# lppllppl920/EndoscopyDepthEstimation-Pytorch

Measured on AMD Instinct MI355X. Metric: train frame-pairs/sec at 256x320 bs=8, higher is better.
Workload: dtype f32

## Files before the change

endoscopydepthestimation-pytorch_amd/csrc/conv_dma_kernels.h:

```cpp
#pragma once

#include "conv_kernels.h"

namespace endo {

static __device__ __attribute__((aligned(16))) float g_pad_consts[8] = {__builtin_nanf(""), __builtin_nanf(""), __builtin_nanf(""), __builtin_nanf(""),
                                                                  0.0f, 0.0f, 0.0f, 0.0f};

typedef const __attribute__((address_space(1))) void* gptr_t;
typedef __attribute__((address_space(3))) void* lptr_t;

template <int KS, int KC, int Q, int WX, int R, int NBUF, int VEC, int IN = IN_PLAIN>
struct ConvDmaSmem {
    using G = ConvGeom<KS, KC, WX, R, VEC>;
    static constexpr int kW = KS * KS * KC * 16 * Q;
    static constexpr int kUG = (G::kTileX / 2) * (G::kTileY / 2);
    static constexpr int kUI = kUG / 4;
    static constexpr int kUStride = ((kUG + kUI - 8 + 31) / 32) * 32 + 8;
    static constexpr int kChan = (IN == IN_UNPOOL) ? kUStride : G::kCS;
    static constexpr int kBuf = KC * kChan + kW;
    static constexpr int kTail = 4 * 16 * Q + 8 * 16 * Q;
    static size_t bytes(int bn_cap) { return sizeof(float) * (NBUF * kBuf + 3 * bn_cap + kTail); }
};

// ... 613 lines not shown
    return launch_dyn(conv_dma_kernel<KS, KC, Q, IN, EPI, WX, R, NBUF, MINW, VEC, XF, EXP, PH, BF>, grid, kConvThreads, S::bytes(p.bn_cap), stream, p);
}

template <int KS, int KC, int Q, int IN, int EPI, int WX, int R, int NBUF, int MINW = 1, int BF = 0>
inline int launch_conv_dma(const ConvParams& p, hipStream_t stream) {
    if constexpr (IN != IN_UPSAMPLE && IN != IN_UNPOOL) {
        const bool aligned = (p.w % 4 == 0) && (p.in_w % 4 == 0) && (p.in_cs % 4 == 0) && (p.in_ns % 4 == 0) &&
                             (reinterpret_cast<uintptr_t>(p.in) % 16 == 0);
        if (aligned) return launch_conv_dma_vec<KS, KC, Q, IN, EPI, WX, R, NBUF, MINW, 4, 0, 0, -1, BF>(p, stream);
    }
    return launch_conv_dma_vec<KS, KC, Q, IN, EPI, WX, R, NBUF, MINW, 1, 0, 0, -1, BF>(p, stream);
}

template <int KS, int KC, int Q, int IN, int EPI, int BIG_R = 8, int NBUF = 2, int BIG_MINW = 1, int BF = 0>
inline int launch_conv_dma_auto(const ConvParams& p, hipStream_t stream) {
    const long tiles_big = static_cast<long>((p.w + 31) / 32) * ((p.h + 15) / 16) * p.n;
    if (tiles_big >= 512) return launch_conv_dma<KS, KC, Q, IN, EPI, 2, BIG_R, NBUF, BIG_MINW, BF>(p, stream);
    const long tiles_mid = static_cast<long>((p.w + 15) / 16) * ((p.h + 15) / 16) * p.n;
    if (tiles_mid >= 384) return launch_conv_dma<KS, KC, Q, IN, EPI, 1, 4, NBUF, 1, BF>(p, stream);
    constexpr int KCS = (NBUF == 2 && KS == 3 && KC <= 8) ? 16 : KC;
    return launch_conv_dma<KS, KCS, Q, IN, EPI, 1, 2, NBUF, 1, BF>(p, stream);
}

}
```

endoscopydepthestimation-pytorch_amd/csrc/conv_kernels.h:

```cpp
#pragma once

#include "common.h"

namespace endo {

enum InMode { IN_PLAIN = 0, IN_BNRELU = 1, IN_UPSAMPLE = 2, IN_UNPOOL = 3, IN_SUBPIX = 4 };
enum Epilogue { EPI_FWD = 0, EPI_FWD_POOL = 1, EPI_DGRAD_BN = 2, EPI_DGRAD_SUMPOOL = 3 };

constexpr int kConvThreads = 256;
constexpr int kMaxBnChannels = 384;

struct ConvParams {
    int n, h, w;
    int tiles_x;
    const float* in;
    int64_t in_ns;
    int in_cs;
    int in_w;
    const uint8_t* in_idx;
    int64_t idx_ns;
    int cin;
    const double* in_sums;
    const float* gamma;
    const float* beta;
// ... 18 lines not shown
    int x_cs;
    const float* bn_saved;
    const float* bn_gamma;
    const float* bn_beta;
    double* bn_scratch;
    int64_t bn_slot_stride;
    int acc_from;
    int bn_cap;
    int ksplit;
    int64_t split_stride;
    int group_n;
    int64_t gs, in_gs, out_gs;
    int sub_c;
    const float* fin_w;
    float* fin_out;
};

__device__ __forceinline__ void group_of(const ConvParams& p, int z, int& grp, int& n) {
    grp = p.group_n > 0 ? z / p.group_n : 0;
    n = z - grp * p.group_n;
}

__device__ __forceinline__ ConvParams group_view(const ConvParams& p, int grp) {
    ConvParams q = p;
    const int64_t o = grp * p.gs;
    q.in += grp * p.in_gs;
    q.out += grp * p.out_gs;
    if (q.x) q.x += o;
    if (q.in_idx) q.in_idx += 4 * o;
    if (q.out_idx) q.out_idx += 4 * o;
    if (q.in_sums) q.in_sums += o / 2;
    if (q.out_sums) q.out_sums += o / 2;
    if (q.bn_scratch) q.bn_scratch += o / 2;
    if (q.saved) q.saved += o;
    if (q.bn_saved) q.bn_saved += o;
    return q;
}

__device__ __forceinline__ void bn_input_constants(const ConvParams& p, const ConvParams& p0, int grp, int groups, bool first_of_group,
                                                   int c, float& scale, float& mean_f, float& beta) {
    double mean, var;
    if (p.training) {
        mean = p.in_sums[2 * c] / p.count;
        var = p.in_sums[2 * c + 1] / p.count - mean * mean;
        if (var < 0.0) var = 0.0;
    } else {
        mean = p.running_mean[c];
        var = p.running_var[c];
    }
    const double rstd = 1.0 / sqrt(var + static_cast<double>(p.eps));
    scale = p.gamma[c] * static_cast<float>(rstd);
    mean_f = static_cast<float>(mean);
    beta = p.beta[c];
    if (first_of_group) {
        if (p.saved) {
            p.saved[2 * c] = static_cast<float>(mean);
            p.saved[2 * c + 1] = static_cast<float>(rstd);
        }
        if (p.training && grp == 0) {
            float rm = p.running_mean[c], rv = p.running_var[c];
            for (int g = 0; g < groups; ++g) {
                const double* sums = p0.in_sums + g * (p0.gs / 2);
                const double m = sums[2 * c] / p.count;
                double v = sums[2 * c + 1] / p.count - m * m;
                if (v < 0.0) v = 0.0;
                const double unbiased = p.count > 1.0 ? v * p.count / (p.count - 1.0) : v;
                rm = (1.0f - p.momentum) * rm + p.momentum * static_cast<float>(m);
                rv = (1.0f - p.momentum) * rv + p.momentum * static_cast<float>(unbiased);
            }
            p.running_mean[c] = rm;
            p.running_var[c] = rv;
        }
    }
}

typedef float f32x4 __attribute__((ext_vector_type(4)));

template <int KS, int KC, int WX, int R, int VEC = 1>
struct ConvGeom {
    static constexpr int kTileX = 16 * WX;
    static constexpr int kTileY = R * (4 / WX);
    static constexpr int kHalo = KS / 2;
    static constexpr int kRows = kTileY + 2 * kHalo;
    static constexpr int kLeft = (VEC == 4 && KS == 3) ? 4 : kHalo;
    static constexpr int kCols = kTileX + 2 * kLeft;
    static constexpr int kColOff = kLeft - kHalo;
    static constexpr int kPlane = kRows * kCols;
// ... 421 lines not shown
```

endoscopydepthestimation-pytorch_amd/csrc/net.hip:

```cpp
#include <new>
#include <vector>

#include "dgrad_kernels.h"
#include "dgrad_block_kernels.h"
#include "dgrad_newmap_kernels.h"
#include "td_dgrad_kernels.h"
#include "td_fwd_kernels.h"
#include "wgrad_taps_kernels.h"
#include "wgrad1x1_kernels.h"
#include "wgrad_nsplit_kernels.h"
#include "wgrad_x3_kernels.h"
#include "wgrad_f34_kernels.h"
#include "wgrad_subpix_kernels.h"
#include "wino_fwd_kernels.h"
#include "wino4_fwd_kernels.h"
#include "dgrad_wino_kernels.h"
#include "dgrad_wino3_kernels.h"


namespace endo {

int run_dgrad_wino3_nl4(const DgradBlockParams& p, const float* const* u, hipStream_t stream);
bool dgrad_wino3p_applies(const DgradBlockParams& p);
int run_dgrad_wino3p_nl4(const DgradBlockParams& p, const float* const* u, int blocks, double* fw_parts, int* blocks_used, hipStream_t stream);

constexpr int kGrowth = 12;
constexpr int kLayers = 4;
constexpr int kFirst = 48;
constexpr int kLevels = 5;
constexpr int kNew = kGrowth * kLayers;
constexpr float kBnEps = 1.0e-5f;
constexpr float kBnMomentum = 0.1f;
constexpr int kSideStreamFromLevel = 0;

struct ConvP { int64_t w, b; int cout, cin, ks; int64_t u; int64_t ud; };
struct BnP { int64_t g, b; int c; int64_t run; int64_t saved; };

struct Table {
    ConvP first, final_;
    ConvP down_conv[kLevels][kLayers], td_conv[kLevels], bott_conv[kLayers], tu_conv[kLevels], up_conv[kLevels][kLayers];
    BnP down_bn[kLevels][kLayers], td_bn[kLevels], bott_bn[kLayers], up_bn[kLevels][kLayers];
    std::vector<int64_t> param_offsets;
    std::vector<BnP*> bn_order;
    int64_t param_floats = 0, bn_floats = 0, bn_width_total = 0;
    WinoWeightTable wino;
    WinoWeightTable wino4;
    int64_t wino4_floats = 0;
// ... 84 lines not shown

struct endo_net {
    int n, h, w;
    int groups;
    int64_t gs;
    struct Level { int h, w, t; int64_t plane; int64_t act, grad; int64_t sums; int64_t pq; } lv[kLevels + 1];
    int64_t pre_off;
    int64_t saved_off;
    int64_t idx_off[kLevels];
    int64_t sums_off;
    int64_t sums_bytes;
    int64_t tape_floats;
    int64_t partial_off;
    int64_t wino_off;
    int64_t wino4_off;
    int64_t pq_off;
    int64_t pq_floats;
    int64_t scratch_off;
    int64_t scratch_bytes;
    int64_t slot_stride;
    int64_t wg_scratch_off;
    int64_t tuw_scratch_off;
    int64_t wd_off;
    int64_t gplane_off;
    int64_t bias_parts_off;
    int64_t fw_parts_off;
    int64_t bias_parts_floats;
    int64_t gradws_floats;
    hipStream_t wstream;
    hipEvent_t ev_fork, ev_join;
// ... 160 lines not shown
            if (training) {
                const double mean = a.saved[j][go + 2 * c], rstd = a.saved[j][go + 2 * c + 1];
                const double scale = a.gamma[j][c] * rstd;
                const double k = scale * rstd * s2 / count;
                dp += static_cast<double>(static_cast<float>(-k));
                dq += static_cast<double>(static_cast<float>(-scale * s1 / count + k * mean));
            }
        }
        if (training) {
            pq_p[c] += static_cast<float>(dp);
            pq_q[c] += static_cast<float>(dq);
        }
    }
}

__global__ void tu_phase_weights_kernel(const float* __restrict__ w, int cout, int cin, float* __restrict__ out) {
    constexpr int kPhW = 2 * 12 * 16 + 16;
    const int total = 2 * cin * 2 * 12 * 16;
    for (int i = blockIdx.x * blockDim.x + threadIdx.x; i < total; i += gridDim.x * blockDim.x) {
        const int lane16 = i & 15;
        const int slot = (i >> 4) % 12;
        const int t = (i / (16 * 12)) & 1;
        const int ci = (i / (16 * 12 * 2)) % cin;
        const int a = i / (16 * 12 * 2 * cin);
        int ctap, tile;
        if (slot < 3) { ctap = 0; tile = slot; } else if (slot < 9) { ctap = 1; tile = slot - 3; } else { ctap = 2; tile = slot - 9 + 3; }
        const int b = tile / 3, co = (tile % 3) * 16 + lane16;
        float v = 0.f;
        if (co < cout) {
            const float* src = w + (static_cast<int64_t>(co) * cin + ci) * 9;
            const int ky0 = a == 0 ? (t == 0 ? 0 : 1) : (t == 0 ? 0 : 2), ky1 = a == 0 ? (t == 0 ? 0 : 2) : (t == 0 ? 1 : 2);
            int kx0, kx1;
// ... 11 lines not shown
    const int total = 4 * cout * 4 * cin;
    for (int i = blockIdx.x * blockDim.x + threadIdx.x; i < total; i += gridDim.x * blockDim.x) {
        const int ci = i % cin;
        const int tap = (i / cin) & 3;
        const int co = (i / (4 * cin)) % cout;
        const int ph = i / (4 * cin * cout);
        const int alpha = ph >> 1, beta = ph & 1, tyi = tap >> 1, txi = tap & 1;
        const int ky0 = alpha == 0 ? (tyi == 0 ? 1 : 0) : (tyi == 0 ? 2 : 0), ky1 = alpha == 0 ? (tyi == 0 ? 2 : 0) : (tyi == 0 ? 2 : 1);
        const int kx0 = beta == 0 ? (txi == 0 ? 1 : 0) : (txi == 0 ? 2 : 0), kx1 = beta == 0 ? (txi == 0 ? 2 : 0) : (txi == 0 ? 2 : 1);
        const float* src = w + (static_cast<int64_t>(co) * cin + ci) * 9;
        float v = 0.f;
        for (int ky = ky0; ky <= ky1; ++ky)
            for (int kx = kx0; kx <= kx1; ++kx) v += src[ky * 3 + kx];
        out[static_cast<int64_t>(ph * cout + co) * pitch + tap * cin + ci] = v;
    }
}

__global__ void __launch_bounds__(256) finalize_partial_kernel(const float* __restrict__ partial, int64_t split_stride, int ksplit,
                                                               int64_t pns, int plane, const float* __restrict__ bias,
                                                               float* __restrict__ out, int64_t out_ns, double* out_sums,
                                                               int group_n, int64_t gs) {
    __shared__ double scratch[2 * 4];
    const int c = blockIdx.y;
    const int grp = blockIdx.z / group_n, n = blockIdx.z - grp * group_n;
    partial += grp * gs; out += grp * gs;
    if (out_sums) out_sums += grp * (gs / 2);
    const float b = bias[c];
    float part[2] = {0.f, 0.f};
    for (int i = blockIdx.x * blockDim.x + threadIdx.x; i < plane; i += gridDim.x * blockDim.x) {
        float v = b;
// ... 112 lines not shown
constexpr int kBlocks = 2 * kLevels + 1, kDense = kBlocks * kLayers;

enum class DenseFwd { Wino4, Wino2_32x16, Wino2_32x8, SplitK, Direct32x8, Direct16x8, DirectAuto };
struct FwdPlan {
    struct Dense {
        DenseFwd form;
        int stages;
        int ksplit;
        bool chunk_weights;
    } dense[kDense];
    bool bf16;
    bool wino4_weights;
    bool fuse_final;
    bool td_persistent[kLevels];
    bool tu_subpix[kLevels];
};

enum class NewMap { Bf16, Persistent, Vec16, Dword };
enum class BasePass { Block8, Block8Bf16, Wino3, Wino3Persistent, Wino8 };
enum class DenseWgrad { F34, X3, NSplit, Taps, Direct };
enum class TdDgrad { Persistent, Runs128, Dma, Staged };
enum class TuWgrad { Subpix, Taps, Direct };
enum class TuDgrad { Subpix32x8, Subpix16x8, Subpix16x4, Plain };
enum class FirstWgrad { F34Prep, F34, Taps, Direct };
struct BwdPlan {
    struct Block {
        bool fused;
        NewMap newmap[kLayers];
        BasePass base;
        bool wino3_layout;
// ... 16 lines not shown
};

struct Ctx {
    const endo_net* net;
    const float* params;
    float* bn_running;
    float* tape;
    float* grads;
    float* gradws;
    int training;
    hipStream_t stream;
    BiasParts* bias_parts = nullptr;
    const float* x = nullptr;
    const FwdPlan* fwd = nullptr;
    const BwdPlan* bwd = nullptr;

    int nt() const { return net->n * net->groups; }
    int fork_wgrad(Ctx& side, int level) const {
        side = *this;
        if (!net->wstream || !bwd->overlap || level < kSideStreamFromLevel) return 0;
        ENDO_CHECK(hipEventRecord(net->ev_fork, stream));
        ENDO_CHECK(hipStreamWaitEvent(net->wstream, net->ev_fork, 0));
        side.stream = net->wstream;
        return 0;
    }
    float* act(int level) const { return tape + net->lv[level].act; }
    float* gbuf(int level) const { return gradws + net->lv[level].grad; }
    double* sums(int level) const { return reinterpret_cast<double*>(reinterpret_cast<char*>(tape) + net->sums_off) + net->lv[level].sums; }
    double* out_sums(int level, int channel) const { return training ? sums(level) + 2 * channel : nullptr; }
    float* saved(const BnP& b) const { return tape + net->saved_off + 2 * b.saved; }
    double* scratch(const BnP& b) const { return reinterpret_cast<double*>(reinterpret_cast<char*>(gradws) + net->scratch_off) + 2 * b.saved; }
    float* pq_p(int level) const { return gradws + net->pq_off + 2 * net->lv[level].pq; }
// ... 27 lines not shown
static void fill_out(const Ctx& c, ConvParams& p, float* base, int level, int oc0, int cout) {
    const auto& lv = c.net->lv[level];
    p.out = base + oc0 * lv.plane;
    p.out_ns = lv.t * lv.plane;
    p.out_cs = static_cast<int>(lv.plane);
    p.out_w = lv.w;
    p.cout = cout;
}

static void fill_grid(const Ctx& c, ConvParams& p, int level) {
    const auto& lv = c.net->lv[level];
    p.n = c.nt(); p.h = lv.h; p.w = lv.w;
    p.group_n = c.net->n; p.gs = c.net->gs; p.in_gs = c.net->gs; p.out_gs = c.net->gs;
}

static double conv_flops(const endo_net* net, int level, int cin, int cout, int ks) {
    return 2.0 * net->n * net->groups * net->lv[level].plane * cin * cout * ks * ks;
}

static void default_options(int (&opt)[ENDO_OPT_COUNT]) {
    opt[ENDO_OPT_WINO_FWD] = 5;
    opt[ENDO_OPT_WINO_DGRAD] = 3;
    opt[ENDO_OPT_DGRAD_VEC] = 2;
    opt[ENDO_OPT_WINO_MIN_TILES] = 1024;
    opt[ENDO_OPT_MFMA_BF16] = 0;
    opt[ENDO_OPT_WGRAD_OVERLAP] = 1;
    opt[ENDO_OPT_MFMA_X3] = 0;
    opt[ENDO_OPT_WGRAD_F34] = 1;
    opt[ENDO_OPT_FINAL_VIRTUAL] = 1;
    opt[ENDO_OPT_TD_PERSIST] = 3;
}
static int bf16_mask(const int* opt) { const int v = opt[ENDO_OPT_MFMA_BF16]; return v == 1 ? 7 : (v >> 1); }

struct DenseBlock { int level, ic0, c0; const BnP* bn; const ConvP* cv; bool base_overwrite; };
static DenseBlock dense_block(int b) {
    const Table& tb = table();
    if (b < kLevels) return {b, 48, down_in(b), tb.down_bn[b], tb.down_conv[b], false};
    if (b == kLevels) return {kLevels, 0, 288, tb.bott_bn, tb.bott_conv, true};
    const int i = b - kLevels - 1, l = kLevels - 1 - i;
    return {l, 0, 96 + down_in(l), tb.up_bn[i], tb.up_conv[i], l > 0};
}
static long tile_count(const Ctx& c, int level, int tx, int ty) {
    const auto& lv = c.net->lv[level];
    return static_cast<long>((lv.w + tx - 1) / tx) * ((lv.h + ty - 1) / ty) * c.nt();
}
// ... 56 lines not shown
            } else if (t32x16 < 512 && t16x16 < 384 && t16x8 < 512 && nchunks >= 4) {
                int want = static_cast<int>(((t16x8 < 256 ? 512 : 768) + t16x8 - 1) / t16x8);
                if (want > nchunks) want = nchunks;
                const int per = (nchunks + want - 1) / want;
                d.form = DenseFwd::SplitK;
                d.ksplit = (nchunks + per - 1) / per;
            } else {
                d.form = (t32x16 < 1024 && t32x8 >= 1024) ? DenseFwd::Direct32x8
                       : (t32x16 < 1024 && t16x8 >= 768) ? DenseFwd::Direct16x8 : DenseFwd::DirectAuto;
            }
        }
    }
    pl.fuse_final = opt[ENDO_OPT_FINAL_VIRTUAL] && pl.dense[kDense - 1].form == DenseFwd::Wino4;
    for (int l = 0; l < kLevels; ++l) {
        pl.td_persistent[l] = (opt[ENDO_OPT_TD_PERSIST] & 2) && !pl.bf16 && c.training && td_fwd_ok(td_fwd_params(c, l));
        const ConvP& tu = table().tu_conv[kLevels - 1 - l];
        pl.tu_subpix[l] = c.net->lv[l + 1].w % 4 == 0 && tu.cout == kNew && tu.cin % 4 == 0;
    }
    return pl;
}

static int dense_fwd(const Ctx& c, int b, int j) {
    const DenseBlock k = dense_block(b);
    const FwdPlan::Dense& d = c.fwd->dense[b * kLayers + j];
    const ConvP& cv = k.cv[j];
    const auto& lv = c.net->lv[k.level];
    const int oc0 = k.ic0 + k.c0 + kGrowth * j;
    ConvParams p = dense_fwd_params(c, k, j, d.form);
    ProfScope prof(kProfConv3x3Dense, c.stream, conv_flops(c.net, k.level, cv.cin, cv.cout, 3),
                   4.0 * c.nt() * lv.plane * (cv.cin + cv.cout));
    const float* chunk_weights = d.chunk_weights ? c.tape + c.net->wino_off + cv.u : nullptr;
    const bool bf16 = c.fwd->bf16;
    switch (d.form) {
        case DenseFwd::Wino4:
            if (c.fwd->fuse_final && b == kBlocks - 1 && j == kLayers - 1) { p.fin_w = c.params + table().final_.w + k.ic0; p.fin_out = c.tape + c.net->pre_off; }
            return launch_wino4_fwd(p, c.stream);
        case DenseFwd::Wino2_32x16:
            return d.stages == 4 ? launch_wino_fwd<2, 4, 2, 4>(p, c.stream) : d.stages == 3 ? launch_wino_fwd<2, 4, 2, 3>(p, c.stream) : launch_wino_fwd<2, 4, 2, 2>(p, c.stream);
        case DenseFwd::Wino2_32x8:
            return d.stages == 4 ? launch_wino_fwd<1, 4, 3, 4>(p, c.stream) : d.stages == 3 ? launch_wino_fwd<1, 4, 3, 3>(p, c.stream) : launch_wino_fwd<1, 4, 3, 2>(p, c.stream);
        case DenseFwd::SplitK: {
            float* partial = c.tape + c.net->partial_off;
            p.ksplit = d.ksplit;
            p.split_stride = static_cast<int64_t>(c.net->n) * cv.cout * lv.plane;
            p.out = partial; p.out_ns = static_cast<int64_t>(cv.cout) * lv.plane;
            p.bias = nullptr; p.out_sums = nullptr;
            p.wgt_chunks = chunk_weights;
            int rc = bf16 ? launch_conv_dma<3, 16, 1, IN_BNRELU, EPI_FWD, 1, 2, 2, 1, 1>(p, c.stream)
                          : launch_conv_dma<3, 16, 1, IN_BNRELU, EPI_FWD, 1, 2, 2, 1>(p, c.stream);
            if (rc) return rc;
            int bx = static_cast<int>((lv.plane + 255) / 256);
            bx = bx > 8 ? 8 : bx;
            finalize_partial_kernel<<<dim3(bx, cv.cout, c.nt()), 256, 0, c.stream>>>(
                partial, p.split_stride, d.ksplit, p.out_ns, static_cast<int>(lv.plane), c.params + cv.b, c.act(k.level) + oc0 * lv.plane,
                lv.t * lv.plane, c.out_sums(k.level, oc0), c.net->n, c.net->gs);
            ENDO_LAUNCH_CHECK();
            return 0;
        }
        case DenseFwd::Direct32x8:
            return bf16 ? launch_conv_dma<3, 4, 1, IN_BNRELU, EPI_FWD, 2, 4, 2, 1, 1>(p, c.stream) : launch_conv_dma<3, 4, 1, IN_BNRELU, EPI_FWD, 2, 4, 2, 1>(p, c.stream);
        case DenseFwd::Direct16x8:
            return bf16 ? launch_conv_dma<3, 8, 1, IN_BNRELU, EPI_FWD, 1, 2, 2, 1, 1>(p, c.stream) : launch_conv_dma<3, 8, 1, IN_BNRELU, EPI_FWD, 1, 2, 2, 1>(p, c.stream);
        case DenseFwd::DirectAuto:
            if (bf16) return launch_conv_dma_auto<3, 4, 1, IN_BNRELU, EPI_FWD, 8, 2, 1, 1>(p, c.stream);
            p.wgt_chunks = chunk_weights;
            return launch_conv_dma_auto<3, 4, 1, IN_BNRELU, EPI_FWD, 8, 2, 1>(p, c.stream);
    }
    return ENDO_E_BADARG;
}

static int td_fwd(const Ctx& c, int level) {
    const ConvP& cv = table().td_conv[level];
    const ConvParams p = td_fwd_params(c, level);
    ProfScope prof(kProfConv1x1Pool, c.stream, conv_flops(c.net, level, cv.cin, cv.cout, 1),
                   4.0 * c.nt() * c.net->lv[level].plane * (cv.cin + cv.cout / 4.0));
    if (c.fwd->td_persistent[level]) return launch_td_fwd(p, device_cu_count(), c.stream);
    if (c.fwd->bf16) return launch_conv_dma_auto<1, 8, 3, IN_BNRELU, EPI_FWD_POOL, 4, 2, 1, 1>(p, c.stream);
    return launch_conv_dma_auto<1, 8, 3, IN_BNRELU, EPI_FWD_POOL, 4>(p, c.stream);
}

static int tu_fwd(const Ctx& c, int level, int src_level, int src_c0, const ConvP& cv) {
    ProfScope prof(kProfConv3x3Up, c.stream, conv_flops(c.net, level, cv.cin, cv.cout, 3),
                   4.0 * c.nt() * c.net->lv[level].plane * (cv.cin / 4.0 + cv.cout));
    if (c.fwd->tu_subpix[level]) {
        float* w3 = c.tape + c.net->partial_off;
        tu_phase_weights_kernel<<<(2 * cv.cin * 384 + 255) / 256, 256, 0, c.stream>>>(c.params + cv.w, cv.cout, cv.cin, w3);
        ENDO_LAUNCH_CHECK();
        ConvParams p{};
        fill_grid(c, p, src_level);
        fill_in(c, p, c.act(src_level), src_level, src_c0, cv.cin);
        p.wgt = w3; p.w_cout = 2 * cv.cout; p.w_cin = cv.cin;
        p.bias = c.params + cv.b;
        fill_out(c, p, c.act(level), level, 0, cv.cout);
        p.out_sums = c.out_sums(level, 0);
        return launch_conv_dma_vec<3, 4, 6, IN_PLAIN, EPI_FWD, 2, 4, 2, 1, 4, 0, 0, 2>(p, c.stream);
    }
    ConvParams p{};
    fill_grid(c, p, level);
    fill_in(c, p, c.act(src_level), src_level, src_c0, cv.cin);
    p.wgt = c.params + cv.w; p.bias = c.params + cv.b; p.w_cout = cv.cout; p.w_cin = cv.cin;
    fill_out(c, p, c.act(level), level, 0, cv.cout);
    p.out_sums = c.out_sums(level, 0);
    return launch_conv_dma_auto<3, 4, 3, IN_UPSAMPLE, EPI_FWD>(p, c.stream);
}

struct FinalVirt { const float* vg; const float* vw; float* gw; };

static int prep_dy(const Ctx& c, int level, int c0, int count, float* bias_grad, const BnFin4* fin = nullptr, int nl = 0, const FinalVirt* fv = nullptr) {
    const auto& lv = c.net->lv[level];
    BnFin4 none{};
    int bx = static_cast<int>((lv.plane + 4095) / 4096);
    bx = bx < 1 ? 1 : (bx > 32 ? 32 : bx);
    float* parts = nullptr;
    if (bias_grad && c.bias_parts) {
        BiasParts& bp = *c.bias_parts;
        const int64_t need = static_cast<int64_t>(count) * c.nt() * bx;
        if (bp.table.n >= kBiasPartLaunches || bp.used + need > c.net->bias_parts_floats) return ENDO_E_UNSUPPORTED;
// ... 464 lines not shown
    net->saved_off = off; off += align_up(2 * tb.bn_width_total, 64);
    int64_t byte_off = off * 4;
    for (int l = 0; l < kLevels; ++l) {
        net->idx_off[l] = byte_off;
        byte_off += align_up(static_cast<int64_t>(n) * (down_in(l) + kNew) * net->lv[l + 1].plane, 256);
    }
    net->sums_off = byte_off;
    net->sums_bytes = sums * 8;
    byte_off += align_up(net->sums_bytes, 256);
    net->partial_off = byte_off / 4;
    byte_off += static_cast<int64_t>(kGrowth) * 163840 * 4;
    net->wino_off = byte_off / 4;
    byte_off += align_up(tb.wino_floats * 4, 256);
    net->wino4_off = byte_off / 4;
    byte_off += align_up(tb.wino4_floats * 4, 256);
    net->tape_floats = byte_off / 4;
    net->pq_off = acts;
    net->pq_floats = 2 * pq;
    net->scratch_off = align_up((acts + net->pq_floats) * 4, 256);
    net->slot_stride = align_up(tb.bn_width_total * 2, 32);
    net->scratch_bytes = net->slot_stride * 8 * kBnSlots;
    net->wg_scratch_off = (net->scratch_off + align_up(net->scratch_bytes, 256)) / 4;
    net->tuw_scratch_off = net->wg_scratch_off + std::max(std::max(kNsScratchFloats, kSpScratchFloats), 4 * kF34ScratchFloats);
    net->wd_off = align_up(net->tuw_scratch_off + 4 * kNew * (4 * kNew + 16), 64);
    net->gplane_off = align_up(net->wd_off + tb.wino_dgrad_floats, 64);
    net->bias_parts_off = net->gplane_off + align_up(static_cast<int64_t>(n) * h * w, 64);
    net->bias_parts_floats = static_cast<int64_t>(kBiasPartChannels) * n * groups * 32;
    {
        int launches = 1, channels = tb.first.cout;
        for (int l = 0; l < kLevels; ++l) {
// ... 53 lines not shown
extern "C" int64_t endo_net_tape_offset(const endo_net* net, int what, int index) {
    if (!net) return -1;
    const Table& tb = table();
    switch (what) {
        case ENDO_TAPE_PRE: return net->pre_off;
        case ENDO_TAPE_BN_SAVED:
            if (index < 0 || index >= static_cast<int>(tb.bn_order.size())) return -1;
            return net->saved_off + 2 * tb.bn_order[index]->saved;
        case ENDO_TAPE_POOL:
            if (index < 0 || index >= kLevels) return -1;
            return net->idx_off[index];
        default: return -1;
    }
}

extern "C" int endo_net_fwd(endo_net* net, const float* params, float* bn_running, const float* x, float* out, float* tape,
                            int training, void* stream_) {
    if (!net || !params || !bn_running || !x || !out || !tape) return ENDO_E_BADARG;
    const Table& tb = table();
    Ctx c{net, params, bn_running, tape, nullptr, nullptr, training, static_cast<hipStream_t>(stream_)};
    const FwdPlan plan = plan_fwd(c);
    c.fwd = &plan;
    for (int g = 0; g < net->groups; ++g)
        ENDO_CHECK(hipMemsetAsync(reinterpret_cast<char*>(tape + g * net->gs) + net->sums_off, 0, net->sums_bytes, c.stream));
    if (!plan.bf16) {
        ProfScope prof(kProfSmall, c.stream, 0.0, 4.0 * (tb.wino_floats + tb.wino_floats * 9 / 16));
        WinoWeightTable wt = tb.wino;
        for (int l = 0; l < wt.layers; ++l) wt.mode[l] = plan.dense[l].chunk_weights ? 1 : 0;
        wino_fwd_weights_kernel<<<(wt.start[wt.layers] + 255) / 256, 256, 0, c.stream>>>(wt, params, tape + net->wino_off);
        ENDO_LAUNCH_CHECK();
        if (plan.wino4_weights) wino4_fwd_weights_kernel<<<(tb.wino4.start[tb.wino4.layers] + 255) / 256, 256, 0, c.stream>>>(tb.wino4, params, tape + net->wino4_off);
        ENDO_LAUNCH_CHECK();
    }
    int rc;
    {
        ConvParams p{};
        fill_grid(c, p, 0);
        p.in = x; p.in_ns = 3 * net->lv[0].plane; p.in_cs = static_cast<int>(net->lv[0].plane); p.in_w = net->w; p.cin = 3;
        p.in_gs = net->n * p.in_ns;
        p.wgt = params + tb.first.w; p.bias = params + tb.first.b; p.w_cout = kFirst; p.w_cin = 3;
        fill_out(c, p, c.act(0), 0, 48, kFirst);
        p.out_sums = c.out_sums(0, 48);
        ProfScope prof(kProfConvFirst, c.stream, conv_flops(net, 0, 3, kFirst, 3), 4.0 * c.nt() * net->lv[0].plane * (3 + kFirst));
        rc = launch_conv_dma_auto<3, 4, 3, IN_PLAIN, EPI_FWD>(p, c.stream);
        if (rc) return rc;
    }
    for (int b = 0; b < kBlocks; ++b) {
        if (b > kLevels) {
            const int i = b - kLevels - 1, l = kLevels - 1 - i;
            rc = tu_fwd(c, l, l + 1, (i == 0) ? 288 : 96 + down_in(l + 1), tb.tu_conv[i]);
            if (rc) return rc;
        }
        for (int j = 0; j < kLayers; ++j) {
            rc = dense_fwd(c, b, j);
            if (rc) return rc;
        }
        if (b < kLevels) {
            rc = td_fwd(c, b);
            if (rc) return rc;
        }
    }
    {
        const auto& lv = net->lv[0];
        const int c_first = plan.fuse_final ? 96 + down_in(0) + kGrowth * (kLayers - 1) : 0;
        ProfScope prof(kProfConvFinal, c.stream, 2.0 * c.nt() * lv.plane * 192, 4.0 * c.nt() * lv.plane * (194 - c_first));
        int bx = static_cast<int>((lv.plane / 4 + 255) / 256);
        bx = bx < 1 ? 1 : bx;
        final_fwd_kernel<<<dim3(bx, c.nt()), 256, 0, c.stream>>>(c.act(0), lv.t * lv.plane, static_cast<int>(lv.plane), 192,
                                                                 params + tb.final_.w, params + tb.final_.b, tape + net->pre_off, out,
                                                                 net->n, net->gs, c_first);
        ENDO_LAUNCH_CHECK();
    }
    return 0;
}

extern "C" int endo_net_bwd(endo_net* net, const float* params, const float* x, const float* tape, const float* grad_out,
                            float* grads, float* gradws, int training, void* stream_) {
    if (!net || !params || !x || !tape || !grad_out || !grads || !gradws) return ENDO_E_BADARG;
    const Table& tb = table();
    Ctx c{net, params, nullptr, const_cast<float*>(tape), grads, gradws, training, static_cast<hipStream_t>(stream_)};
    c.x = x;
    const BwdPlan plan = plan_bwd(c);
    c.bwd = &plan;
    BiasParts bias_parts{};
    c.bias_parts = &bias_parts;
    if (!net->wstream) {
        ENDO_CHECK(hipStreamCreateWithFlags(&net->wstream, hipStreamNonBlocking));
        ENDO_CHECK(hipEventCreateWithFlags(&net->ev_fork, hipEventDisableTiming));
        ENDO_CHECK(hipEventCreateWithFlags(&net->ev_join, hipEventDisableTiming));
    }
    for (int g = 0; g < net->groups; ++g)
        ENDO_CHECK(hipMemsetAsync(gradws + g * net->gs + net->pq_off, 0,
                                  static_cast<size_t>(net->scratch_off + net->scratch_bytes - net->pq_off * 4), c.stream));
    if (plan.dgrad_weights) {
        ProfScope prof(kProfSmall, c.stream, 0.0, 4.0 * 2.0 * tb.wino_dgrad_floats);
        int layout1_blocks = 0;
        for (int b = 0; b < kBlocks; ++b) layout1_blocks |= plan.block[b].wino3_layout ? 1 << b : 0;
        dgrad_wino_weights_kernel<<<(tb.wino_dgrad.start[tb.wino_dgrad.layers] + 255) / 256, 256, 0, c.stream>>>(tb.wino_dgrad, params, gradws + net->wd_off, layout1_blocks);
        ENDO_LAUNCH_CHECK();
    }
    int rc;
    const FinalVirt virt{gradws + net->gplane_off, params + tb.final_.w, grads + tb.final_.w};
    {
        const auto& lv = net->lv[0];
// ... 75 lines not shown
```

endoscopydepthestimation-pytorch_amd/models.py:

```python

import ctypes

import torch
from torch import nn

from . import _lib

GROWTH = 12
LAYERS = 4
FIRST = 48
LEVELS = 5


class ConvParams(nn.Module):

    def __init__(self, cin, cout, k):
        super().__init__()
        self.weight = nn.Parameter(torch.empty(cout, cin, k, k))
        self.bias = nn.Parameter(torch.zeros(cout))
        nn.init.kaiming_uniform_(self.weight, a=5 ** 0.5)


class FusedBatchNorm2d(nn.Module):

# ... 218 lines not shown
                p.grad = self._flat_grad[off:off + p.numel()].view(p.shape)

    def _handle(self, n, h, w, groups=1):
        key = (n, h, w, groups)
        if key not in self._handles:
            lib = _lib.load()
            if lib.endo_net_param_floats() != self._flat.numel():
                raise RuntimeError("parameter packing mismatch between Python and libendo_hip.so")
            hnd = ctypes.c_void_p()
            _lib.check(lib.endo_net_create_grouped(ctypes.byref(hnd), n, h, w, groups), "endo_net_create_grouped(%d,%d,%d,%d)" % key)
            for option_id, value in getattr(self, "_kernel_options", {}).items():
                lib.endo_net_set_option(hnd, option_id, value)
            self._handles[key] = (hnd, int(lib.endo_net_tape_floats(hnd)), int(lib.endo_net_gradws_floats(hnd)))
        return self._handles[key]

    _OPTION_DEFAULTS = {0: 5, 1: 3, 2: 2, 3: 1024, 4: 0, 5: 1, 6: 0, 7: 1, 8: 1, 9: 3}

    def set_kernel_option(self, option_id, value):
        option_id, value = int(option_id), int(value)
        if option_id not in self._OPTION_DEFAULTS:
            raise ValueError("unknown kernel option %d" % option_id)
        options = self.__dict__.setdefault("_kernel_options", {})
        old = options.get(option_id, self._OPTION_DEFAULTS[option_id])
        options[option_id] = value
        lib = _lib.load()
        for key, (hnd, _, _) in self._handles.items():
            if key[0] in ("bf16", "fp16"):
                continue
            rc = lib.endo_net_set_option(hnd, option_id, value)
            if rc < 0:
                raise RuntimeError("endo_net_set_option(%d, %d) failed: %d" % (option_id, value, rc))
# ... 334 lines not shown
```

include/endo_hip.h:

```cpp
#ifndef ENDO_HIP_H
#define ENDO_HIP_H

#include <stdint.h>

#ifdef __cplusplus
extern "C" {
#endif

#define ENDO_E_BADARG (-1)
#define ENDO_E_UNSUPPORTED (-2)

#define ENDO_ABI_VERSION 6
int endo_abi_version(void);
const char* endo_error_string(int code);

int endo_depth_scale_fwd(const float* pred, const float* sparse_depth, const float* sparse_mask,
                         float* scaled, float* ratio, double* stats,
                         int n, int hw, float eps, void* stream);
int endo_depth_scale_bwd(const float* grad_scaled, const float* grad_ratio,
                         const float* pred, const float* sparse_depth, const double* stats,
                         float* grad_pred, double* work,
                         int n, int hw, float eps, void* stream);

int endo_flow_from_depth_fwd(const float* depth, const float* mask, const float* t, const float* R,
// ... 66 lines not shown
typedef struct endo_net endo_net;

int endo_net_create(endo_net** out, int n, int h, int w);
int endo_net_create_grouped(endo_net** out, int n, int h, int w, int groups);
int endo_net_groups(const endo_net* net);
#define ENDO_OPT_WINO_FWD 0
#define ENDO_OPT_WINO_DGRAD 1
#define ENDO_OPT_DGRAD_VEC 2
#define ENDO_OPT_WINO_MIN_TILES 3
#define ENDO_OPT_MFMA_BF16 4
#define ENDO_OPT_WGRAD_OVERLAP 5
#define ENDO_OPT_MFMA_X3 6
#define ENDO_OPT_WGRAD_F34 7
#define ENDO_OPT_FINAL_VIRTUAL 8
#define ENDO_OPT_TD_PERSIST 9
#define ENDO_OPT_COUNT 10
int endo_net_set_option(endo_net* net, int option_id, int value);
int endo_net_get_option(const endo_net* net, int option_id);
int64_t endo_net_group_stride(const endo_net* net);
void endo_net_destroy(endo_net* net);
int64_t endo_net_param_floats(void);
int64_t endo_net_bn_floats(void);
int64_t endo_net_tape_floats(const endo_net* net);
int64_t endo_net_gradws_floats(const endo_net* net);
int64_t endo_net_param_offset(int index);
int64_t endo_net_bn_offset(int bn_index, int which );

int endo_net_fwd(endo_net* net, const float* params, float* bn_running, const float* x, float* out,
                 float* tape, int training, void* stream);
int endo_net_bwd(endo_net* net, const float* params, const float* x, const float* tape,
                 const float* grad_out, float* grads, float* gradws, int training, void* stream);
// ... 124 lines not shown
```

Measured before the change: 512.1.

## Fork grouped forward into per-group stream chains and batch TU phase weight prep

```diff
diff --git a/endoscopydepthestimation-pytorch_amd/csrc/conv_dma_kernels.h b/endoscopydepthestimation-pytorch_amd/csrc/conv_dma_kernels.h
--- a/endoscopydepthestimation-pytorch_amd/csrc/conv_dma_kernels.h
+++ b/endoscopydepthestimation-pytorch_amd/csrc/conv_dma_kernels.h
@@ -651,9 +651,10 @@
 
 template <int KS, int KC, int Q, int IN, int EPI, int BIG_R = 8, int NBUF = 2, int BIG_MINW = 1, int BF = 0>
 inline int launch_conv_dma_auto(const ConvParams& p, hipStream_t stream) {
-    const long tiles_big = static_cast<long>((p.w + 31) / 32) * ((p.h + 15) / 16) * p.n;
+    const int plan_n = p.plan_n > 0 ? p.plan_n : p.n;
+    const long tiles_big = static_cast<long>((p.w + 31) / 32) * ((p.h + 15) / 16) * plan_n;
     if (tiles_big >= 512) return launch_conv_dma<KS, KC, Q, IN, EPI, 2, BIG_R, NBUF, BIG_MINW, BF>(p, stream);
-    const long tiles_mid = static_cast<long>((p.w + 15) / 16) * ((p.h + 15) / 16) * p.n;
+    const long tiles_mid = static_cast<long>((p.w + 15) / 16) * ((p.h + 15) / 16) * plan_n;
     if (tiles_mid >= 384) return launch_conv_dma<KS, KC, Q, IN, EPI, 1, 4, NBUF, 1, BF>(p, stream);
     constexpr int KCS = (NBUF == 2 && KS == 3 && KC <= 8) ? 16 : KC;
     return launch_conv_dma<KS, KCS, Q, IN, EPI, 1, 2, NBUF, 1, BF>(p, stream);
diff --git a/endoscopydepthestimation-pytorch_amd/csrc/conv_kernels.h b/endoscopydepthestimation-pytorch_amd/csrc/conv_kernels.h
--- a/endoscopydepthestimation-pytorch_amd/csrc/conv_kernels.h
+++ b/endoscopydepthestimation-pytorch_amd/csrc/conv_kernels.h
@@ -56,6 +56,7 @@
     int sub_c;
     const float* fin_w;
     float* fin_out;
+    int plan_n;
 };
 
 __device__ __forceinline__ void group_of(const ConvParams& p, int z, int& grp, int& n) {
@@ -79,6 +80,22 @@
     return q;
 }
 
+__device__ __forceinline__ void bn_running_update(float* running_mean, float* running_var, const double* sums0, int64_t gs2, int groups, int c,
+                                                  double count, float momentum) {
+    float rm = running_mean[c], rv = running_var[c];
+    for (int g = 0; g < groups; ++g) {
+        const double* sums = sums0 + g * gs2;
+        const double m = sums[2 * c] / count;
+        double v = sums[2 * c + 1] / count - m * m;
+        if (v < 0.0) v = 0.0;
+        const double unbiased = count > 1.0 ? v * count / (count - 1.0) : v;
+        rm = (1.0f - momentum) * rm + momentum * static_cast<float>(m);
+        rv = (1.0f - momentum) * rv + momentum * static_cast<float>(unbiased);
+    }
+    running_mean[c] = rm;
+    running_var[c] = rv;
+}
+
 __device__ __forceinline__ void bn_input_constants(const ConvParams& p, const ConvParams& p0, int grp, int groups, bool first_of_group,
                                                    int c, float& scale, float& mean_f, float& beta) {
     double mean, var;
@@ -99,20 +116,8 @@
             p.saved[2 * c] = static_cast<float>(mean);
             p.saved[2 * c + 1] = static_cast<float>(rstd);
         }
-        if (p.training && grp == 0) {
-            float rm = p.running_mean[c], rv = p.running_var[c];
-            for (int g = 0; g < groups; ++g) {
-                const double* sums = p0.in_sums + g * (p0.gs / 2);
-                const double m = sums[2 * c] / p.count;
-                double v = sums[2 * c + 1] / p.count - m * m;
-                if (v < 0.0) v = 0.0;
-                const double unbiased = p.count > 1.0 ? v * p.count / (p.count - 1.0) : v;
-                rm = (1.0f - p.momentum) * rm + p.momentum * static_cast<float>(m);
-                rv = (1.0f - p.momentum) * rv + p.momentum * static_cast<float>(unbiased);
-            }
-            p.running_mean[c] = rm;
-            p.running_var[c] = rv;
-        }
+        if (p.training && grp == 0 && p.running_mean)
+            bn_running_update(p.running_mean, p.running_var, p0.in_sums, p0.gs / 2, groups, c, p.count, p.momentum);
     }
 }
 
diff --git a/endoscopydepthestimation-pytorch_amd/csrc/net.hip b/endoscopydepthestimation-pytorch_amd/csrc/net.hip
--- a/endoscopydepthestimation-pytorch_amd/csrc/net.hip
+++ b/endoscopydepthestimation-pytorch_amd/csrc/net.hip
@@ -31,6 +31,7 @@
 constexpr int kNew = kGrowth * kLayers;
 constexpr float kBnEps = 1.0e-5f;
 constexpr float kBnMomentum = 0.1f;
+constexpr long kForkMaxTiles = 2048;
 constexpr int kSideStreamFromLevel = 0;
 
 struct ConvP { int64_t w, b; int cout, cin, ks; int64_t u; int64_t ud; };
@@ -145,6 +146,7 @@
     int64_t partial_off;
     int64_t wino_off;
     int64_t wino4_off;
+    int64_t tuw_off[kLevels];
     int64_t pq_off;
     int64_t pq_floats;
     int64_t scratch_off;
@@ -335,8 +337,12 @@
     }
 }
 
-__global__ void tu_phase_weights_kernel(const float* __restrict__ w, int cout, int cin, float* __restrict__ out) {
+struct TuPhaseTable { int count; int cout[kLevels], cin[kLevels]; int64_t w_off[kLevels], out_off[kLevels]; };
+__global__ void tu_phase_weights_kernel(const TuPhaseTable tab, const float* __restrict__ params, float* __restrict__ tape) {
     constexpr int kPhW = 2 * 12 * 16 + 16;
+    const int cout = tab.cout[blockIdx.y], cin = tab.cin[blockIdx.y];
+    const float* w = params + tab.w_off[blockIdx.y];
+    float* out = tape + tab.out_off[blockIdx.y];
     const int total = 2 * cin * 2 * 12 * 16;
     for (int i = blockIdx.x * blockDim.x + threadIdx.x; i < total; i += gridDim.x * blockDim.x) {
         const int lane16 = i & 15;
@@ -378,6 +384,16 @@
             for (int kx = kx0; kx <= kx1; ++kx) v += src[ky * 3 + kx];
         out[static_cast<int64_t>(ph * cout + co) * pitch + tap * cin + ci] = v;
     }
+}
+
+constexpr int kBnRunLayers = 48;
+struct BnRunTable { int count; int c[kBnRunLayers]; int64_t sums[kBnRunLayers], run[kBnRunLayers]; double n[kBnRunLayers]; };
+__global__ void __launch_bounds__(256) bn_running_update_kernel(const BnRunTable tab, const double* __restrict__ sums0, int64_t gs2, int groups,
+                                                                float* __restrict__ bn_running, float momentum) {
+    const int e = blockIdx.x;
+    float* rm = bn_running + tab.run[e];
+    for (int c = threadIdx.x; c < tab.c[e]; c += blockDim.x)
+        bn_running_update(rm, rm + tab.c[e], sums0 + tab.sums[e], gs2, groups, c, tab.n[e], momentum);
 }
 
 __global__ void __launch_bounds__(256) finalize_partial_kernel(const float* __restrict__ partial, int64_t split_stride, int ksplit,
@@ -520,6 +536,7 @@
     bool fuse_final;
     bool td_persistent[kLevels];
     bool tu_subpix[kLevels];
+    int fork_level;
 };
 
 enum class NewMap { Bf16, Persistent, Vec16, Dword };
@@ -566,8 +583,11 @@
     const float* x = nullptr;
     const FwdPlan* fwd = nullptr;
     const BwdPlan* bwd = nullptr;
+    int grp = -1;
 
     int nt() const { return net->n * net->groups; }
+    int ln() const { return grp >= 0 ? net->n : nt(); }
+    double share() const { return grp >= 0 ? 1.0 / net->groups : 1.0; }
     int fork_wgrad(Ctx& side, int level) const {
         side = *this;
         if (!net->wstream || !bwd->overlap || level < kSideStreamFromLevel) return 0;
@@ -625,6 +645,21 @@
     p.group_n = c.net->n; p.gs = c.net->gs; p.in_gs = c.net->gs; p.out_gs = c.net->gs;
 }
 
+static void chain_view(const Ctx& c, ConvParams& p) {
+    if (c.grp < 0) return;
+    const int64_t o = c.grp * p.gs;
+    p.in += c.grp * p.in_gs;
+    p.out += c.grp * p.out_gs;
+    if (p.out_idx) p.out_idx += 4 * o;
+    if (p.in_sums) p.in_sums += o / 2;
+    if (p.out_sums) p.out_sums += o / 2;
+    if (p.saved) p.saved += o;
+    if (p.fin_out) p.fin_out += o;
+    p.plan_n = p.n;
+    p.n = c.net->n;
+    if (p.training) { p.running_mean = nullptr; p.running_var = nullptr; }
+}
+
 static double conv_flops(const endo_net* net, int level, int cin, int cout, int ks) {
     return 2.0 * net->n * net->groups * net->lv[level].plane * cin * cout * ks * ks;
 }
@@ -640,6 +675,7 @@
     opt[ENDO_OPT_WGRAD_F34] = 1;
     opt[ENDO_OPT_FINAL_VIRTUAL] = 1;
     opt[ENDO_OPT_TD_PERSIST] = 3;
+    opt[ENDO_OPT_FWD_FORK] = 0;
 }
 static int bf16_mask(const int* opt) { const int v = opt[ENDO_OPT_MFMA_BF16]; return v == 1 ? 7 : (v >> 1); }
 
@@ -726,8 +762,14 @@
     pl.fuse_final = opt[ENDO_OPT_FINAL_VIRTUAL] && pl.dense[kDense - 1].form == DenseFwd::Wino4;
     for (int l = 0; l < kLevels; ++l) {
         pl.td_persistent[l] = (opt[ENDO_OPT_TD_PERSIST] & 2) && !pl.bf16 && c.training && td_fwd_ok(td_fwd_params(c, l));
-        const ConvP& tu = table().tu_conv[kLevels - 1 - l];
-        pl.tu_subpix[l] = c.net->lv[l + 1].w % 4 == 0 && tu.cout == kNew && tu.cin % 4 == 0;
+        pl.tu_subpix[l] = c.net->tuw_off[l] >= 0;
+    }
+    const int fork = opt[ENDO_OPT_FWD_FORK];
+    pl.fork_level = 0;
+    if (c.net->groups == 2 && !pl.bf16 && opt[ENDO_OPT_WGRAD_OVERLAP] != 0) {
+        if (fork >= 12 && fork <= 10 + kLevels) pl.fork_level = fork - 10;
+        if (fork == 1)
+            for (int l = kLevels; l >= 2 && tile_count(c, l, 16, 8) < kForkMaxTiles; --l) pl.fork_level = l;
     }
     return pl;
 }
@@ -739,17 +781,20 @@
     const auto& lv = c.net->lv[k.level];
     const int oc0 = k.ic0 + k.c0 + kGrowth * j;
     ConvParams p = dense_fwd_params(c, k, j, d.form);
-    ProfScope prof(kProfConv3x3Dense, c.stream, conv_flops(c.net, k.level, cv.cin, cv.cout, 3),
-                   4.0 * c.nt() * lv.plane * (cv.cin + cv.cout));
+    ProfScope prof(kProfConv3x3Dense, c.stream, conv_flops(c.net, k.level, cv.cin, cv.cout, 3) * c.share(),
+                   4.0 * c.ln() * lv.plane * (cv.cin + cv.cout));
     const float* chunk_weights = d.chunk_weights ? c.tape + c.net->wino_off + cv.u : nullptr;
     const bool bf16 = c.fwd->bf16;
     switch (d.form) {
         case DenseFwd::Wino4:
             if (c.fwd->fuse_final && b == kBlocks - 1 && j == kLayers - 1) { p.fin_w = c.params + table().final_.w + k.ic0; p.fin_out = c.tape + c.net->pre_off; }
+            chain_view(c, p);
             return launch_wino4_fwd(p, c.stream);
         case DenseFwd::Wino2_32x16:
+            chain_view(c, p);
             return d.stages == 4 ? launch_wino_fwd<2, 4, 2, 4>(p, c.stream) : d.stages == 3 ? launch_wino_fwd<2, 4, 2, 3>(p, c.stream) : launch_wino_fwd<2, 4, 2, 2>(p, c.stream);
         case DenseFwd::Wino2_32x8:
+            chain_view(c, p);
             return d.stages == 4 ? launch_wino_fwd<1, 4, 3, 4>(p, c.stream) : d.stages == 3 ? launch_wino_fwd<1, 4, 3, 3>(p, c.stream) : launch_wino_fwd<1, 4, 3, 2>(p, c.stream);
         case DenseFwd::SplitK: {
             float* partial = c.tape + c.net->partial_off;
@@ -758,24 +803,30 @@
             p.out = partial; p.out_ns = static_cast<int64_t>(cv.cout) * lv.plane;
             p.bias = nullptr; p.out_sums = nullptr;
             p.wgt_chunks = chunk_weights;
+            chain_view(c, p);
             int rc = bf16 ? launch_conv_dma<3, 16, 1, IN_BNRELU, EPI_FWD, 1, 2, 2, 1, 1>(p, c.stream)
                           : launch_conv_dma<3, 16, 1, IN_BNRELU, EPI_FWD, 1, 2, 2, 1>(p, c.stream);
             if (rc) return rc;
             int bx = static_cast<int>((lv.plane + 255) / 256);
             bx = bx > 8 ? 8 : bx;
-            finalize_partial_kernel<<<dim3(bx, cv.cout, c.nt()), 256, 0, c.stream>>>(
-                partial, p.split_stride, d.ksplit, p.out_ns, static_cast<int>(lv.plane), c.params + cv.b, c.act(k.level) + oc0 * lv.plane,
-                lv.t * lv.plane, c.out_sums(k.level, oc0), c.net->n, c.net->gs);
+            const int64_t go = c.grp >= 0 ? c.grp * c.net->gs : 0;
+            double* out_sums = c.out_sums(k.level, oc0);
+            finalize_partial_kernel<<<dim3(bx, cv.cout, c.ln()), 256, 0, c.stream>>>(
+                partial + go, p.split_stride, d.ksplit, p.out_ns, static_cast<int>(lv.plane), c.params + cv.b, c.act(k.level) + oc0 * lv.plane + go,
+                lv.t * lv.plane, out_sums ? out_sums + go / 2 : nullptr, c.net->n, c.net->gs);
             ENDO_LAUNCH_CHECK();
             return 0;
         }
         case DenseFwd::Direct32x8:
+            chain_view(c, p);
             return bf16 ? launch_conv_dma<3, 4, 1, IN_BNRELU, EPI_FWD, 2, 4, 2, 1, 1>(p, c.stream) : launch_conv_dma<3, 4, 1, IN_BNRELU, EPI_FWD, 2, 4, 2, 1>(p, c.stream);
         case DenseFwd::Direct16x8:
+            chain_view(c, p);
             return bf16 ? launch_conv_dma<3, 8, 1, IN_BNRELU, EPI_FWD, 1, 2, 2, 1, 1>(p, c.stream) : launch_conv_dma<3, 8, 1, IN_BNRELU, EPI_FWD, 1, 2, 2, 1>(p, c.stream);
         case DenseFwd::DirectAuto:
             if (bf16) return launch_conv_dma_auto<3, 4, 1, IN_BNRELU, EPI_FWD, 8, 2, 1, 1>(p, c.stream);
             p.wgt_chunks = chunk_weights;
+            chain_view(c, p);
             return launch_conv_dma_auto<3, 4, 1, IN_BNRELU, EPI_FWD, 8, 2, 1>(p, c.stream);
     }
     return ENDO_E_BADARG;
@@ -783,21 +834,20 @@
 
 static int td_fwd(const Ctx& c, int level) {
     const ConvP& cv = table().td_conv[level];
-    const ConvParams p = td_fwd_params(c, level);
-    ProfScope prof(kProfConv1x1Pool, c.stream, conv_flops(c.net, level, cv.cin, cv.cout, 1),
-                   4.0 * c.nt() * c.net->lv[level].plane * (cv.cin + cv.cout / 4.0));
+    ConvParams p = td_fwd_params(c, level);
+    chain_view(c, p);
+    ProfScope prof(kProfConv1x1Pool, c.stream, conv_flops(c.net, level, cv.cin, cv.cout, 1) * c.share(),
+                   4.0 * c.ln() * c.net->lv[level].plane * (cv.cin + cv.cout / 4.0));
     if (c.fwd->td_persistent[level]) return launch_td_fwd(p, device_cu_count(), c.stream);
     if (c.fwd->bf16) return launch_conv_dma_auto<1, 8, 3, IN_BNRELU, EPI_FWD_POOL, 4, 2, 1, 1>(p, c.stream);
     return launch_conv_dma_auto<1, 8, 3, IN_BNRELU, EPI_FWD_POOL, 4>(p, c.stream);
 }
 
 static int tu_fwd(const Ctx& c, int level, int src_level, int src_c0, const ConvP& cv) {
-    ProfScope prof(kProfConv3x3Up, c.stream, conv_flops(c.net, level, cv.cin, cv.cout, 3),
-                   4.0 * c.nt() * c.net->lv[level].plane * (cv.cin / 4.0 + cv.cout));
+    ProfScope prof(kProfConv3x3Up, c.stream, conv_flops(c.net, level, cv.cin, cv.cout, 3) * c.share(),
+                   4.0 * c.ln() * c.net->lv[level].plane * (cv.cin / 4.0 + cv.cout));
     if (c.fwd->tu_subpix[level]) {
-        float* w3 = c.tape + c.net->partial_off;
-        tu_phase_weights_kernel<<<(2 * cv.cin * 384 + 255) / 256, 256, 0, c.stream>>>(c.params + cv.w, cv.cout, cv.cin, w3);
-        ENDO_LAUNCH_CHECK();
+        const float* w3 = c.tape + c.net->tuw_off[level];
         ConvParams p{};
         fill_grid(c, p, src_level);
         fill_in(c, p, c.act(src_level), src_level, src_c0, cv.cin);
@@ -805,6 +855,7 @@
         p.bias = c.params + cv.b;
         fill_out(c, p, c.act(level), level, 0, cv.cout);
         p.out_sums = c.out_sums(level, 0);
+        chain_view(c, p);
         return launch_conv_dma_vec<3, 4, 6, IN_PLAIN, EPI_FWD, 2, 4, 2, 1, 4, 0, 0, 2>(p, c.stream);
     }
     ConvParams p{};
@@ -813,6 +864,7 @@
     p.wgt = c.params + cv.w; p.bias = c.params + cv.b; p.w_cout = cv.cout; p.w_cin = cv.cin;
     fill_out(c, p, c.act(level), level, 0, cv.cout);
     p.out_sums = c.out_sums(level, 0);
+    chain_view(c, p);
     return launch_conv_dma_auto<3, 4, 3, IN_UPSAMPLE, EPI_FWD>(p, c.stream);
 }
 
@@ -1307,6 +1359,12 @@
     byte_off += align_up(tb.wino_floats * 4, 256);
     net->wino4_off = byte_off / 4;
     byte_off += align_up(tb.wino4_floats * 4, 256);
+    for (int l = 0; l < kLevels; ++l) {
+        const ConvP& tu = tb.tu_conv[kLevels - 1 - l];
+        const bool subpix = net->lv[l + 1].w % 4 == 0 && tu.cout == kNew && tu.cin % 4 == 0;
+        net->tuw_off[l] = subpix ? byte_off / 4 : -1;
+        if (subpix) byte_off += align_up(static_cast<int64_t>(2) * tu.cin * 400 * 4, 256);
+    }
     net->tape_floats = byte_off / 4;
     net->pq_off = acts;
     net->pq_floats = 2 * pq;
@@ -1390,6 +1448,14 @@
     }
 }
 
+static int ensure_side_stream(endo_net* net) {
+    if (net->wstream) return 0;
+    ENDO_CHECK(hipStreamCreateWithFlags(&net->wstream, hipStreamNonBlocking));
+    ENDO_CHECK(hipEventCreateWithFlags(&net->ev_fork, hipEventDisableTiming));
+    ENDO_CHECK(hipEventCreateWithFlags(&net->ev_join, hipEventDisableTiming));
+    return 0;
+}
+
 extern "C" int endo_net_fwd(endo_net* net, const float* params, float* bn_running, const float* x, float* out, float* tape,
                             int training, void* stream_) {
     if (!net || !params || !bn_running || !x || !out || !tape) return ENDO_E_BADARG;
@@ -1408,6 +1474,22 @@
         if (plan.wino4_weights) wino4_fwd_weights_kernel<<<(tb.wino4.start[tb.wino4.layers] + 255) / 256, 256, 0, c.stream>>>(tb.wino4, params, tape + net->wino4_off);
         ENDO_LAUNCH_CHECK();
     }
+    {
+        TuPhaseTable tt{};
+        int max_cin = 0;
+        for (int l = 0; l < kLevels; ++l) {
+            if (!plan.tu_subpix[l]) continue;
+            const ConvP& cv = tb.tu_conv[kLevels - 1 - l];
+            const int e = tt.count++;
+            tt.cout[e] = cv.cout; tt.cin[e] = cv.cin; tt.w_off[e] = cv.w; tt.out_off[e] = net->tuw_off[l];
+            max_cin = cv.cin > max_cin ? cv.cin : max_cin;
+        }
+        if (tt.count > 0) {
+            ProfScope prof(kProfSmall, c.stream, 0.0, 4.0 * tt.count * max_cin * (9.0 * kNew + 2 * 384));
+            tu_phase_weights_kernel<<<dim3((2 * max_cin * 384 + 255) / 256, tt.count), 256, 0, c.stream>>>(tt, params, tape);
+            ENDO_LAUNCH_CHECK();
+        }
+    }
     int rc;
     {
         ConvParams p{};
@@ -1421,19 +1503,53 @@
         rc = launch_conv_dma_auto<3, 4, 3, IN_PLAIN, EPI_FWD>(p, c.stream);
         if (rc) return rc;
     }
-    for (int b = 0; b < kBlocks; ++b) {
+    auto block = [&](int b, const Ctx* cs, int count) -> int {
+        int rc = 0;
         if (b > kLevels) {
             const int i = b - kLevels - 1, l = kLevels - 1 - i;
-            rc = tu_fwd(c, l, l + 1, (i == 0) ? 288 : 96 + down_in(l + 1), tb.tu_conv[i]);
+            for (int k = 0; k < count && !rc; ++k) rc = tu_fwd(cs[k], l, l + 1, (i == 0) ? 288 : 96 + down_in(l + 1), tb.tu_conv[i]);
+        }
+        for (int j = 0; j < kLayers; ++j)
+            for (int k = 0; k < count && !rc; ++k) rc = dense_fwd(cs[k], b, j);
+        if (b < kLevels)
+            for (int k = 0; k < count && !rc; ++k) rc = td_fwd(cs[k], b);
+        return rc;
+    };
+    const int fork_first = plan.fork_level, fork_last = 2 * kLevels - plan.fork_level;
+    for (int b = 0; b < kBlocks; ++b) {
+        if (fork_first == 0 || b != fork_first) {
+            rc = block(b, &c, 1);
             if (rc) return rc;
-        }
-        for (int j = 0; j < kLayers; ++j) {
-            rc = dense_fwd(c, b, j);
-            if (rc) return rc;
-        }
-        if (b < kLevels) {
-            rc = td_fwd(c, b);
-            if (rc) return rc;
+            continue;
+        }
+        rc = ensure_side_stream(net);
+        if (rc) return rc;
+        ENDO_CHECK(hipEventRecord(net->ev_fork, c.stream));
+        ENDO_CHECK(hipStreamWaitEvent(net->wstream, net->ev_fork, 0));
+        Ctx chain[2] = {c, c};
+        chain[0].grp = 0;
+        chain[1].grp = 1; chain[1].stream = net->wstream;
+        for (; b <= fork_last && !rc; ++b) rc = block(b, chain, 2);
+        b = fork_last;
+        const hipError_t e1 = hipEventRecord(net->ev_join, net->wstream);
+        const hipError_t e2 = e1 == hipSuccess ? hipStreamWaitEvent(c.stream, net->ev_join, 0) : e1;
+        if (rc) return rc;
+        ENDO_CHECK(e2);
+        if (training) {
+            BnRunTable rt{};
+            auto add = [&](const BnP& bn, int level, int ic0) {
+                const int e = rt.count++;
+                rt.c[e] = bn.c; rt.sums[e] = net->lv[level].sums + 2 * ic0; rt.run[e] = bn.run;
+                rt.n[e] = static_cast<double>(net->n) * net->lv[level].h * net->lv[level].w;
+            };
+            for (int r = fork_first; r <= fork_last; ++r) {
+                const DenseBlock k = dense_block(r);
+                for (int j = 0; j < kLayers; ++j) add(k.bn[j], k.level, k.ic0);
+                if (r < kLevels) add(tb.td_bn[r], r, 48);
+            }
+            ProfScope prof(kProfSmall, c.stream, 0.0, 0.0);
+            bn_running_update_kernel<<<rt.count, 256, 0, c.stream>>>(rt, c.sums(0) - net->lv[0].sums, net->gs / 2, net->groups, bn_running, kBnMomentum);
+            ENDO_LAUNCH_CHECK();
         }
     }
     {
@@ -1460,10 +1576,9 @@
     c.bwd = &plan;
     BiasParts bias_parts{};
     c.bias_parts = &bias_parts;
-    if (!net->wstream) {
-        ENDO_CHECK(hipStreamCreateWithFlags(&net->wstream, hipStreamNonBlocking));
-        ENDO_CHECK(hipEventCreateWithFlags(&net->ev_fork, hipEventDisableTiming));
-        ENDO_CHECK(hipEventCreateWithFlags(&net->ev_join, hipEventDisableTiming));
+    {
+        const int rc = ensure_side_stream(net);
+        if (rc) return rc;
     }
     for (int g = 0; g < net->groups; ++g)
         ENDO_CHECK(hipMemsetAsync(gradws + g * net->gs + net->pq_off, 0,
diff --git a/endoscopydepthestimation-pytorch_amd/models.py b/endoscopydepthestimation-pytorch_amd/models.py
--- a/endoscopydepthestimation-pytorch_amd/models.py
+++ b/endoscopydepthestimation-pytorch_amd/models.py
@@ -256,7 +256,7 @@
             self._handles[key] = (hnd, int(lib.endo_net_tape_floats(hnd)), int(lib.endo_net_gradws_floats(hnd)))
         return self._handles[key]
 
-    _OPTION_DEFAULTS = {0: 5, 1: 3, 2: 2, 3: 1024, 4: 0, 5: 1, 6: 0, 7: 1, 8: 1, 9: 3}
+    _OPTION_DEFAULTS = {0: 5, 1: 3, 2: 2, 3: 1024, 4: 0, 5: 1, 6: 0, 7: 1, 8: 1, 9: 3, 10: 0}
 
     def set_kernel_option(self, option_id, value):
         option_id, value = int(option_id), int(value)
diff --git a/include/endo_hip.h b/include/endo_hip.h
--- a/include/endo_hip.h
+++ b/include/endo_hip.h
@@ -104,7 +104,8 @@
 #define ENDO_OPT_WGRAD_F34 7
 #define ENDO_OPT_FINAL_VIRTUAL 8
 #define ENDO_OPT_TD_PERSIST 9
-#define ENDO_OPT_COUNT 10
+#define ENDO_OPT_FWD_FORK 10
+#define ENDO_OPT_COUNT 11
 int endo_net_set_option(endo_net* net, int option_id, int value);
 int endo_net_get_option(const endo_net* net, int option_id);
 int64_t endo_net_group_stride(const endo_net* net);
```

New measurement: 513.9, median of 3. About the same (+0.4%).
